# myungsub/meta-interpolation

Measured on AMD Instinct MI355X. Metric: inner-loop steps/sec, higher is better.
Workload: dtype f32 (3x3 convolutions: Winograd F(4x4) / F(2x2) on exact-f32 MFMAs, csrc/winograd4.h + winograd.hip; weight gradients and 5x5 / 7x7 / direct layers on csrc/convk*.hip: bf16x6 split operands, f32 accumulate; 51-tap op on 8-bit frames: exact integer frames x bf16x3 split taps, f32 accumulate); 1 GPU; c2_sepconv_256x448_b4_s5; plugin=sepconv, tasks_per_gpu=4, global_meta_batch=4, inner_steps=5, frame=256x448x3, inner_rule=lslr+SGD, seeded_weights=default, parallelism=task-parallel x1, 1 all-reduce of outer grads

## Files before the change

meta-interpolation_amd/csrc/winograd4.h:

```cpp
#pragma once

namespace w4 {

constexpr int TT = 32;
constexpr int COB = 32;
constexpr int KC = 8;
constexpr int PTS = 36;
constexpr int VBUF = PTS * KC * TT;
constexpr int XBUF = PTS * 16 * TT;
constexpr int LDS_FLOATS = XBUF > 2 * VBUF ? XBUF : 2 * VBUF;
#ifndef SAVFI_W4_MAXC
#define SAVFI_W4_MAXC 512
#endif

__host__ __device__ inline bool use_f4(int K, int I) { return K <= SAVFI_W4_MAXC && I <= SAVFI_W4_MAXC; }
__host__ __device__ inline int kp_of(int K) { return (K + KC - 1) / KC * KC; }
__host__ __device__ inline int ip_of(int I) { return (I + COB - 1) / COB * COB; }

__device__ __forceinline__ void g_rows(const float (&g)[3], float (&t)[6]) {
  const float s = g[0] + g[2];
  const float s4 = fmaf(4.f, g[2], g[0]);
  t[0] = 0.25f * g[0];
  t[1] = (s + g[1]) * (-1.f / 6.f);
  t[2] = (s - g[1]) * (-1.f / 6.f);
  t[3] = fmaf(2.f, g[1], s4) * (1.f / 24.f);
  t[4] = fmaf(-2.f, g[1], s4) * (1.f / 24.f);
  t[5] = g[2];
}

__device__ __forceinline__ void filter_transform_block4(const float* __restrict__ w, float* __restrict__ U, int Co, int Ci, int K, int I,
                                                        int KP, int IP, int mode, int bx, int by) {
  __shared__ __attribute__((aligned(16))) float stage[8 * 18 * 64];
  const int kk = threadIdx.x & 3, ii = threadIdx.x >> 2;
  const int nI = (IP + 63) / 64;
  const int k = 4 * bx + kk, i = 64 * (by % nI) + ii;
  const int task = by / nI;
  w += (size_t)task * Co * Ci * 9;
  U += (size_t)task * PTS * KP * IP;
  float g[3][3];
#pragma unroll
  for (int a = 0; a < 3; ++a)
#pragma unroll
    for (int b = 0; b < 3; ++b) {
      float val = 0.f;
      if (k < K && i < I)
        val = mode == 0 ? w[((size_t)i * Ci + k) * 9 + a * 3 + b] : w[((size_t)k * Ci + i) * 9 + (2 - a) * 3 + (2 - b)];
      g[a][b] = val;
    }
  float t[6][3];
#pragma unroll
  for (int b = 0; b < 3; ++b) {
    const float col[3] = {g[0][b], g[1][b], g[2][b]};
    float o[6];
    g_rows(col, o);
#pragma unroll
    for (int r = 0; r < 6; ++r) t[r][b] = o[r];
  }
  const int cbl = ii >> 5, cb = (ii >> 4) & 1, il = ii & 15;
  const int lane = kk * 16 + il;
#pragma unroll
  for (int r = 0; r < 6; ++r) {
    float o[6];
    g_rows(t[r], o);
#pragma unroll
    for (int c = 0; c < 6; ++c) {
      const int xi = 6 * r + c, wave = xi / 9, v = 2 * (xi % 9) + cb;
      float* blk = stage + (cbl * 4 + wave) * (18 * 64);
      if (v < 16) blk[((v >> 2) * 64 + lane) * 4 + (v & 3)] = o[c];
      else blk[16 * 64 + lane * 2 + (v - 16)] = o[c];
    }
  }
  __syncthreads();
  const int chunk = bx >> 1, s2 = bx & 1, ncob = IP / COB, cob0 = 2 * (by % nI);
  if (4 * bx >= KP) return;
#pragma unroll
  for (int it = 0; it < 8 * 18 * 64 / 4 / 256; ++it) {
    const int e = (it * 256 + threadIdx.x) * 4;
    const int blkid = e / (18 * 64), off = e - blkid * (18 * 64);
    const int cobq = cob0 + (blkid >> 2), wv = blkid & 3;
    if (cobq >= ncob) continue;
    float* dst = U + ((((size_t)chunk * ncob + cobq) * 4 + wv) * 2 + s2) * (18 * 64) + off;
    *reinterpret_cast<f32x4*>(dst) = *reinterpret_cast<const f32x4*>(stage + e);
  }
}

struct W4Args {
  const float* x;
  const float* U;
  const float* bias;
  float* out;
  int K, I, KP, IP, H, W, Ho, Wo, off, tiles_y, tiles_x;
  float slope;
  int tile_shift;
  int T, N;
  const float* mask;
  float mask_slope;
  int out_unit16;
  int nsplit, chunks_per_split;
  float* partial;
  int flat, ty4, tx4, ntb;
  unsigned tx_mul;
  float* pooled;
  int Hp, Wp;
};

__device__ __forceinline__ i32x4 w4_rsrc(const void* base, unsigned bytes) {
  const unsigned long long p = reinterpret_cast<unsigned long long>(base);
  i32x4 r;
  r.x = (int)(unsigned)p;
  r.y = (int)(unsigned)(p >> 32);
  r.z = (int)bytes;
  r.w = 0x00020000;
  return r;
}

__device__ __forceinline__ i32x4 w4_uniform(i32x4 r) {
  r.x = __builtin_amdgcn_readfirstlane(r.x); r.y = __builtin_amdgcn_readfirstlane(r.y);
  r.z = __builtin_amdgcn_readfirstlane(r.z); r.w = __builtin_amdgcn_readfirstlane(r.w);
  return r;
}

__device__ __forceinline__ void bt6(float d0, float d1, float d2, float d3, float d4, float d5, float (&o)[6]) {
  const float a = fmaf(-4.f, d2, d4), b = fmaf(-4.f, d1, d3);
  const float c = d4 - d2, e = d3 - d1;
  o[0] = fmaf(4.f, d0, fmaf(-5.f, d2, d4));
  o[1] = a + b;
  o[2] = a - b;
  o[3] = fmaf(2.f, e, c);
  o[4] = fmaf(-2.f, e, c);
  o[5] = fmaf(4.f, d1, fmaf(-5.f, d3, d5));
}

__device__ __forceinline__ f32x2 w4_fma2(float s, f32x2 x, f32x2 y) { return __builtin_elementwise_fma((f32x2){s, s}, x, y); }
__device__ __forceinline__ void bt6p(f32x2 d0, f32x2 d1, f32x2 d2, f32x2 d3, f32x2 d4, f32x2 d5, f32x2 (&o)[6]) {
  const f32x2 a = w4_fma2(-4.f, d2, d4), b = w4_fma2(-4.f, d1, d3);
  const f32x2 c = d4 - d2, e = d3 - d1;
  o[0] = w4_fma2(4.f, d0, w4_fma2(-5.f, d2, d4));
  o[1] = a + b;
  o[2] = a - b;
  o[3] = w4_fma2(2.f, e, c);
  o[4] = w4_fma2(-2.f, e, c);
  o[5] = w4_fma2(4.f, d1, w4_fma2(-5.f, d3, d5));
}

__device__ __forceinline__ void at6(float m0, float m1, float m2, float m3, float m4, float m5, float (&o)[4]) {
  const float s1 = m1 + m2, d1 = m1 - m2, s2 = m3 + m4, d2 = m3 - m4;
  o[0] = m0 + s1 + s2;
  o[1] = fmaf(2.f, d2, d1);
  o[2] = fmaf(4.f, s2, s1);
  o[3] = fmaf(8.f, d2, d1) + m5;
}

__device__ __forceinline__ void at6p(f32x2 m0, f32x2 m1, f32x2 m2, f32x2 m3, f32x2 m4, f32x2 m5, f32x2 (&o)[4]) {
  const f32x2 s1 = m1 + m2, d1 = m1 - m2, s2 = m3 + m4, d2 = m3 - m4;
  o[0] = m0 + s1 + s2;
  o[1] = w4_fma2(2.f, d2, d1);
  o[2] = w4_fma2(4.f, s2, s1);
  o[3] = w4_fma2(8.f, d2, d1) + m5;
}

template <int VECW, int IN16, bool MASK, bool POOL = false>
__global__ __launch_bounds__(256, 2) void wino4_conv3x3(W4Args a) {
  extern __shared__ __attribute__((aligned(16))) float lds[];
  const int tid = threadIdx.x, lane = tid & 63, w = __builtin_amdgcn_readfirstlane(tid >> 6);
  const int j = lane & 15, kg = lane >> 4;

  const int nblk = a.IP / COB;
  int tb, cob, n, sp;
  {
    const unsigned flat = blockIdx.x, nwg = gridDim.x;
    const unsigned ntb = (unsigned)a.ntb;
    const unsigned xcd = flat & 7u, q8 = nwg >> 3, rem = nwg & 7u;
    unsigned item = xcd * q8 + min(xcd, rem) + (flat >> 3);
    cob = (int)(item % (unsigned)nblk);
    item /= (unsigned)nblk;
    tb = (int)(item % ntb);
    item /= ntb;
    sp = (int)(item % (unsigned)a.nsplit);
    n = (int)(item / (unsigned)a.nsplit);
  }
  const int i0 = cob * COB;
  const int task = a.T > 1 ? n % a.T : 0;
  const size_t cplane = (size_t)a.H * a.W;
  const float* xp = a.x + (size_t)n * a.K * cplane;

  const int tl = lane & 31;
  auto tile_of = [&](int tbq, int& ty, int& tx) {
    if (a.flat) {
      const unsigned t = 32u * (unsigned)tbq + (unsigned)tl, tx4 = (unsigned)a.tx4;
      unsigned q = __umulhi(t, a.tx_mul);
      unsigned r = t - q * tx4;
      if (r >= tx4) { ++q; r -= tx4; }
      ty = (int)q;
      tx = (int)r;
      return t < (unsigned)a.ty4 * tx4;
    }
    const int tsh = a.tile_shift, tbw = 1 << tsh, tbh = TT >> tsh;
    const int tby = tbq / a.tiles_x, tbx = tbq - tby * a.tiles_x;
    ty = tby * tbh + (tl >> tsh);
    tx = tbx * tbw + (tl & (tbw - 1));
    return true;
  };

  const int kc = 2 * w + (lane >> 5);
  int tyi, txi;
  const bool live = tile_of(tb, tyi, txi);
  const int y0 = live ? 4 * tyi - a.off : a.H, x0 = live ? 4 * txi - a.off : 0;
  constexpr int WC = IN16 ? IN16 - 1 : 0;
  unsigned pv[6], pn[IN16 ? 6 : 1], pn2[IN16 == 2 ? 6 : 1];
  unsigned long long shl = 0, colm[6] = {~0ull, ~0ull, ~0ull, ~0ull, ~0ull, ~0ull};
  int partial = 0;
  unsigned chunk_bytes;
  unsigned plane_b;
  if constexpr (IN16) {
    plane_b = 64u;
    chunk_bytes = KC * 64u;
    auto at = [&](bool row, int y, int x) {
      return (row && x >= 0 && x < a.W) ? (unsigned)((y * (a.W >> 4) + (x >> 4)) * a.K) * 64u + (unsigned)(x & 15) * 4u + (unsigned)kc * 64u : 0x80000000u;
    };
#pragma unroll
    for (int r = 0; r < 6; ++r) {
      const int y = y0 + r;
      const bool row = y >= 0 && y < a.H;
      pv[r] = at(row, y, x0 + WC);
      pn[IN16 ? r : 0] = at(row, y, x0);
      if constexpr (IN16 == 2) pn2[r] = at(row, y, x0 + 5);
    }
  } else {
    plane_b = (unsigned)cplane * 4u;
    chunk_bytes = KC * plane_b;
    const int xa = x0 < 0 ? 0 : x0;
#pragma unroll
    for (int r = 0; r < 6; ++r) {
      const int y = y0 + r;
      pv[r] = (y >= 0 && y < a.H) ? (unsigned)(y * a.W + xa) * 4u + (unsigned)kc * plane_b : 0x80000000u;
    }
    shl = __builtin_amdgcn_ballot_w64(x0 < 0);
    const unsigned long long all = __builtin_amdgcn_ballot_w64(true);
#pragma unroll
    for (int c = 0; c < 6; ++c) {
      colm[c] = __builtin_amdgcn_ballot_w64(!live || (x0 + c >= 0 && x0 + c < a.W));
      if (colm[c] != all) partial |= 1 << c;
    }
  }
  const int cbeg = sp * a.chunks_per_split;
  const int nch = min(cbeg + a.chunks_per_split, a.KP / KC) - cbeg;
  const unsigned sample_bytes = (unsigned)a.K * (unsigned)cplane * 4u;
  auto xrs = [&](int c) {
    c = (c < nch - 1 ? c : nch - 1) + cbeg;
    const unsigned first = (unsigned)c * chunk_bytes;
    return w4_rsrc(reinterpret_cast<const char*>(xp) + first, sample_bytes - first);
  };

  float d[6][6];
  auto load_wide = [&](const i32x4& rs) {
#pragma unroll
    for (int r = 0; r < 6; ++r) {
      const f32x4 v = savfi_raw_buffer_load_x4(rs, (int)pv[r], 0, 0);
      d[r][WC] = v.x; d[r][WC + 1] = v.y; d[r][WC + 2] = v.z; d[r][WC + 3] = v.w;
    }
  };
  auto load_narrow = [&](const i32x4& rs) {
#pragma unroll
    for (int r = 0; r < 6; ++r) {
      if constexpr (IN16 == 3) {
        const f32x2 v = savfi_raw_buffer_load_x2(rs, (int)pn[r], 0, 0);
        d[r][0] = v.x; d[r][1] = v.y;
      } else if constexpr (IN16 == 2) {
        d[r][0] = savfi_raw_buffer_load_x1(rs, (int)pn[r], 0, 0);
        d[r][5] = savfi_raw_buffer_load_x1(rs, (int)pn2[r], 0, 0);
      } else {
        const f32x2 v = savfi_raw_buffer_load_x2(rs, (int)pv[r] + 16, 0, 0);
        d[r][4] = v.x; d[r][5] = v.y;
      }
    }
  };
  const bool edge = !IN16 && (shl != 0 || partial != 0);
  auto fix_patch = [&]() {
    if (shl != 0) {
      if (a.off == 1) {
#pragma unroll
        for (int r = 0; r < 6; ++r)
#pragma unroll
          for (int c = 5; c >= 1; --c) asm volatile("v_cndmask_b32 %0, %0, %1, %2" : "+v"(d[r][c]) : "v"(d[r][c - 1]), "s"(shl));
      } else if (a.off == 2) {
#pragma unroll
        for (int r = 0; r < 6; ++r)
#pragma unroll
          for (int c = 5; c >= 2; --c) asm volatile("v_cndmask_b32 %0, %0, %1, %2" : "+v"(d[r][c]) : "v"(d[r][c - 2]), "s"(shl));
      }
    }
#pragma unroll
    for (int c = 0; c < 6; ++c)
      if (partial & (1 << c)) {
#pragma unroll
        for (int r = 0; r < 6; ++r) asm volatile("v_cndmask_b32 %0, 0, %0, %1" : "+v"(d[r][c]) : "s"(colm[c]));
      }
  };
  const int vw = (((kc >> 2) * 4 + (kc & 3)) * 16 + (tl & 15)) * 2 + (tl >> 4);
  f32x2 tp[6][3];
  auto pk_cols = [&](int cp) {
    f32x2 o[6];
    bt6p((f32x2){d[0][2 * cp], d[0][2 * cp + 1]}, (f32x2){d[1][2 * cp], d[1][2 * cp + 1]}, (f32x2){d[2][2 * cp], d[2][2 * cp + 1]},
         (f32x2){d[3][2 * cp], d[3][2 * cp + 1]}, (f32x2){d[4][2 * cp], d[4][2 * cp + 1]}, (f32x2){d[5][2 * cp], d[5][2 * cp + 1]}, o);
#pragma unroll
    for (int r = 0; r < 6; ++r) tp[r][cp] = o[r];
  };
  auto row_out = [&](int rp, float* vdst) {
    float o[6];
    bt6(tp[rp][0].x, tp[rp][0].y, tp[rp][1].x, tp[rp][1].y, tp[rp][2].x, tp[rp][2].y, o);
#pragma unroll
    for (int c = 0; c < 6; ++c) vdst[vw + (6 * rp + c) * 256] = o[c];
  };
  auto load_row = [&](const i32x4& rs, int r) {
    const f32x4 v = savfi_raw_buffer_load_x4(rs, (int)pv[r], 0, 0);
    d[r][WC] = v.x; d[r][WC + 1] = v.y; d[r][WC + 2] = v.z; d[r][WC + 3] = v.w;
    if constexpr (IN16 == 3) {
      const f32x2 u = savfi_raw_buffer_load_x2(rs, (int)pn[r], 0, 0);
      d[r][0] = u.x; d[r][1] = u.y;
    } else if constexpr (IN16 == 2) {
      d[r][0] = savfi_raw_buffer_load_x1(rs, (int)pn[r], 0, 0);
      d[r][5] = savfi_raw_buffer_load_x1(rs, (int)pn2[r], 0, 0);
    } else {
      const f32x2 u = savfi_raw_buffer_load_x2(rs, (int)pv[r] + 16, 0, 0);
      d[r][4] = u.x; d[r][5] = u.y;
    }
  };

  f32x4 acc[9][2][2];
#pragma unroll
  for (int q = 0; q < 9; ++q)
#pragma unroll
    for (int cb = 0; cb < 2; ++cb)
#pragma unroll
      for (int t = 0; t < 2; ++t) acc[q][cb][t] = (f32x4){0.f, 0.f, 0.f, 0.f};
  const unsigned ubytes = (unsigned)PTS * (unsigned)a.KP * (unsigned)a.IP * 4u;
  const i32x4 urs = w4_rsrc(a.U + (size_t)task * PTS * a.KP * a.IP, ubytes);
  const unsigned ulane4 = (unsigned)lane * 16u, ulane2 = 16u * 64u * 4u + (unsigned)lane * 8u;
  auto u_of = [&](int c, int s) {
    c = (c < nch - 1 ? c : nch - 1) + cbeg;
    return ((((unsigned)c * (unsigned)nblk + (unsigned)cob) * 4u + (unsigned)w) * 2u + (unsigned)s) * (18u * 64u * 4u);
  };
  f32x4 a4[4];
  f32x2 a2;
  auto load_a4 = [&](int b, unsigned uo) { a4[b] = savfi_raw_buffer_load_x4(urs, (int)(ulane4 + (unsigned)b * 1024u), (int)uo, 0); };
  auto load_a2 = [&](unsigned uo) { a2 = savfi_raw_buffer_load_x2(urs, (int)ulane2, (int)uo, 0); };
  const int vr = (9 * w * 8 + kg) * 32 + 2 * j;

  {
    const i32x4 rs = xrs(0);
    load_wide(rs);
    load_narrow(rs);
  }
  load_a4(0, u_of(0, 0)); load_a4(1, u_of(0, 0)); load_a4(2, u_of(0, 0)); load_a4(3, u_of(0, 0)); load_a2(u_of(0, 0));
  if (edge) fix_patch();
#pragma unroll
  for (int cp = 0; cp < 3; ++cp) pk_cols(cp);
#pragma unroll
  for (int r = 0; r < 6; ++r) row_out(r, lds);
  {
    const i32x4 rs = xrs(1);
    load_wide(rs);
    load_narrow(rs);
  }
  __builtin_amdgcn_s_waitcnt(0);
  __syncthreads();

  const bool half_last = cbeg + nch == a.KP / KC && a.K - (a.KP - KC) <= 4;
  auto chunk = [&](int ch, const float* vcur, float* vnext, auto last_tag) {
    constexpr bool last = decltype(last_tag)::value;
    f32x2 bq[3];
    bq[0] = *reinterpret_cast<const f32x2*>(vcur + vr);
    bq[1] = *reinterpret_cast<const f32x2*>(vcur + vr + 256);
    const i32x4 rs2 = xrs(ch + 2);
#pragma unroll
    for (int g = 0; g < 18; ++g) {
      const int s = g / 9, q = g % 9;
      if (last && g == 9 && half_last) break;
      if (g + 2 < 18) {
        const int s2 = (g + 2) / 9, q2 = (g + 2) % 9;
        bq[(g + 2) % 3] = *reinterpret_cast<const f32x2*>(vcur + vr + q2 * 256 + s2 * 128);
      }
#pragma unroll
      for (int cb = 0; cb < 2; ++cb) {
        const int v = 2 * q + cb;
        const float av = v < 16 ? a4[v >> 2][v & 3] : a2[v - 16];
#pragma unroll
        for (int t = 0; t < 2; ++t) {
          acc[q][cb][t] = __builtin_amdgcn_mfma_f32_16x16x4f32(av, bq[g % 3][t], acc[q][cb][t], 0, 0, 0);
        }
      }
      const unsigned un = s == 0 ? u_of(ch, 1) : u_of(ch + 1, 0);
      if (q == 1 || q == 3 || q == 5 || q == 7) load_a4(q >> 1, un);
      if (q == 8) load_a2(un);
      if (!last) {
        if (g == 9 && edge) fix_patch();
        if (g >= 9 && g < 12) pk_cols(g - 9);
        if (g >= 12) { row_out(g - 12, vnext); load_row(rs2, g - 12); }
      }
      __builtin_amdgcn_sched_barrier(0);
    }
  };
  for (int ch = 0; ch < nch - 1; ++ch) {
    const int cur = ch & 1;
    chunk(ch, lds + cur * VBUF, lds + (cur ^ 1) * VBUF, std::false_type{});
    __syncthreads();
  }
  chunk(nch - 1, lds + ((nch - 1) & 1) * VBUF, lds, std::true_type{});
  __builtin_amdgcn_s_waitcnt(0);
  __syncthreads();

  const int split = a.nsplit > 1 ? 1 : 0;
  float* const obase = split ? a.partial + (size_t)sp * a.N * a.I * a.Ho * a.Wo : a.out;
  float bvals[2][2];
#pragma unroll
  for (int cb = 0; cb < 2; ++cb)
#pragma unroll
    for (int qq = 0; qq < 2; ++qq) {
      const int i = i0 + 16 * cb + (tid >> 5) + 8 * qq;
      bvals[cb][qq] = (a.bias && split == 0 && i < a.I) ? a.bias[task * a.I + i] : 0.f;
    }

  const int otl = tid & 31, och = tid >> 5;
  int tbo = tb, oty = tyi, otx = txi;
  bool olive = live;
  if constexpr (!MASK) {
    asm volatile("" : "+s"(tbo));
    olive = tile_of(tbo, oty, otx);
  }
  const int oy = olive ? 4 * oty : a.Ho, ox = 4 * otx;
  const unsigned oplane = (unsigned)(a.Ho * a.Wo) * 4u;
  constexpr int NS = 4 / VECW;
  unsigned ooff[4][NS];
#pragma unroll
  for (int r = 0; r < 4; ++r)
#pragma unroll
    for (int e = 0; e < NS; ++e) {
      const int x = ox + e * VECW;
      const bool ok = oy + r < a.Ho && x < a.Wo;
      if (a.out_unit16) ooff[r][e] = ok ? (unsigned)(((oy + r) * (a.Wo >> 4) + (x >> 4)) * a.I) * 64u + (unsigned)(x & 15) * 4u : 0x80000000u;
      else ooff[r][e] = ok ? (unsigned)((oy + r) * a.Wo + x) * 4u + (unsigned)(lane >> 5) * oplane : 0x80000000u;
    }
  auto pair_rsrc = [&](const float* base, int cb, int qq, unsigned plane_bytes = 0) {
    if (plane_bytes == 0) plane_bytes = oplane;
    const int ie = i0 + 16 * cb + 2 * w + 8 * qq;
    const int have = a.I - ie < 0 ? 0 : (a.I - ie > 2 ? 2 : a.I - ie);
    return w4_rsrc(base + ((size_t)n * a.I + (ie < a.I ? ie : 0)) * (plane_bytes >> 2), (unsigned)have * plane_bytes);
  };
  constexpr int PS = VECW == 4 ? 1 : 2;
  const unsigned pplane = POOL ? (unsigned)(a.Hp * a.Wp) * 4u : 0u;
  unsigned poff[POOL ? 2 : 1][POOL ? PS : 1];
  if constexpr (POOL) {
#pragma unroll
    for (int r = 0; r < 2; ++r)
#pragma unroll
      for (int e = 0; e < PS; ++e) {
        const int py = (oy >> 1) + r, px = (ox >> 1) + e;
        poff[r][e] = (py < a.Hp && px < a.Wp) ? (unsigned)(py * a.Wp + px) * 4u + (unsigned)(lane >> 5) * pplane : 0x80000000u;
      }
  }
  float mk[MASK ? 2 : 1][MASK ? 2 : 1][4][4];
  if constexpr (MASK) {
#pragma unroll
    for (int cb = 0; cb < 2; ++cb)
#pragma unroll
      for (int qq = 0; qq < 2; ++qq) {
        const i32x4 mrs = w4_uniform(pair_rsrc(a.mask, cb, qq));
#pragma unroll
        for (int r = 0; r < 4; ++r)
#pragma unroll
          for (int e = 0; e < NS; ++e) {
            if constexpr (VECW == 4) {
              const f32x4 v = savfi_raw_buffer_load_x4(mrs, (int)ooff[r][e], 0, 0);
              mk[cb][qq][r][0] = v.x; mk[cb][qq][r][1] = v.y; mk[cb][qq][r][2] = v.z; mk[cb][qq][r][3] = v.w;
            } else if constexpr (VECW == 2) {
              const f32x2 v = savfi_raw_buffer_load_x2(mrs, (int)ooff[r][e], 0, 0);
              mk[cb][qq][r][2 * e] = v.x; mk[cb][qq][r][2 * e + 1] = v.y;
            } else {
              mk[cb][qq][r][e] = savfi_raw_buffer_load_x1(mrs, (int)ooff[r][e], 0, 0);
            }
          }
      }
  }
  const float slope = a.slope;
#pragma unroll
  for (int cb = 0; cb < 2; ++cb) {
#pragma unroll
    for (int q = 0; q < 9; ++q)
#pragma unroll
      for (int t = 0; t < 2; ++t)
#pragma unroll
        for (int r = 0; r < 4; ++r)
          lds[((9 * w + q) * 16 + 4 * kg + r) * 32 + ((16 * t + j) ^ (16 * (kg & 1)))] = acc[q][cb][t][r];
    __syncthreads();
    auto finish = [&](auto act_tag) {
      constexpr int ACT = decltype(act_tag)::value;
#pragma unroll
      for (int qq = 0; qq < 2; ++qq) {
        const int chl = och + 8 * qq;
        const int col = otl ^ (16 * ((chl >> 2) & 1));
        f32x2 t4p[4][3];
#pragma unroll
        for (int cp = 0; cp < 3; ++cp) {
          f32x2 m[6], o[4];
#pragma unroll
          for (int r = 0; r < 6; ++r)
            m[r] = (f32x2){lds[((6 * r + 2 * cp) * 16 + chl) * 32 + col], lds[((6 * r + 2 * cp + 1) * 16 + chl) * 32 + col]};
          at6p(m[0], m[1], m[2], m[3], m[4], m[5], o);
#pragma unroll
          for (int r = 0; r < 4; ++r) t4p[r][cp] = o[r];
        }
        const float b = bvals[cb][qq];
        const int i = i0 + 16 * cb + chl;
        const i32x4 ors = w4_uniform(a.out_unit16 ? w4_rsrc(obase + (size_t)n * a.I * a.Ho * a.Wo, (unsigned)a.I * oplane) : pair_rsrc(obase, cb, qq));
        const unsigned choff = a.out_unit16 ? (i < a.I ? (unsigned)i * 64u : 0x40000000u) : 0u;
        i32x4 prs = ors;
        if constexpr (POOL) prs = w4_uniform(pair_rsrc(a.pooled, cb, qq, pplane));
        float ye[4];
#pragma unroll
        for (int r = 0; r < 4; ++r) {
          float y[4];
          at6(t4p[r][0].x, t4p[r][0].y, t4p[r][1].x, t4p[r][1].y, t4p[r][2].x, t4p[r][2].y, y);
#pragma unroll
          for (int c = 0; c < 4; ++c) {
            float v = y[c];
            if constexpr (ACT >= 1) v += b;
            if constexpr (ACT == 2) v = fmaxf(v, 0.f);
            if constexpr (ACT == 3) v = fmaxf(v, 0.f) + slope * fminf(v, 0.f);
            if constexpr (MASK) v = mk[MASK ? cb : 0][MASK ? qq : 0][r][c] > 0.f ? v : v * a.mask_slope;
            y[c] = v;
          }
          if constexpr (VECW == 4) {
            savfi_raw_buffer_store_x4((f32x4){y[0], y[1], y[2], y[3]}, ors, (int)(ooff[r][0] + choff), 0, 0);
          } else if constexpr (VECW == 2) {
            savfi_raw_buffer_store_x2((f32x2){y[0], y[1]}, ors, (int)(ooff[r][0] + choff), 0, 0);
            savfi_raw_buffer_store_x2((f32x2){y[2], y[3]}, ors, (int)(ooff[r][1] + choff), 0, 0);
          } else {
#pragma unroll
            for (int c = 0; c < 4; ++c) savfi_raw_buffer_store_x1(y[c], ors, (int)(ooff[r][c] + choff), 0, 0);
          }
          if constexpr (POOL) {
            if (r % 2 == 0) {
#pragma unroll
              for (int c = 0; c < 4; ++c) ye[c] = y[c];
            } else {
              const float p0 = (((ye[0] + ye[1]) + y[0]) + y[1]) / 4.f, p1 = (((ye[2] + ye[3]) + y[2]) + y[3]) / 4.f;
              if constexpr (VECW == 4) {
                savfi_raw_buffer_store_x2((f32x2){p0, p1}, prs, (int)poff[r >> 1][0], 0, 0);
              } else {
                savfi_raw_buffer_store_x1(p0, prs, (int)poff[r >> 1][0], 0, 0);
                savfi_raw_buffer_store_x1(p1, prs, (int)poff[r >> 1][1], 0, 0);
              }
            }
          }
        }
      }
    };
    if (slope == 1.f || split) {
      if (a.bias == nullptr || split) finish(std::integral_constant<int, 0>{});
      else finish(std::integral_constant<int, 1>{});
    } else if (slope == 0.f) {
      finish(std::integral_constant<int, 2>{});
    } else {
      finish(std::integral_constant<int, 3>{});
    }
    __syncthreads();
  }
}

}
```

Measured before the change: 250.0 inner-loop steps/sec.

## Restructure Winograd F(4x4) epilogue to exchange accumulators via wave-partitioned LDS transpose

Result: faster. 252.6 inner-loop steps/sec (median of 6 runs) (+1.0%).

```diff
diff --git a/meta-interpolation_amd/csrc/winograd4.h b/meta-interpolation_amd/csrc/winograd4.h
--- a/meta-interpolation_amd/csrc/winograd4.h
+++ b/meta-interpolation_amd/csrc/winograd4.h
@@ -185,9 +185,9 @@
   const float* xp = a.x + (size_t)n * a.K * cplane;
 
   const int tl = lane & 31;
-  auto tile_of = [&](int tbq, int& ty, int& tx) {
+  auto tile_of = [&](int tbq, int slot, int& ty, int& tx) {
     if (a.flat) {
-      const unsigned t = 32u * (unsigned)tbq + (unsigned)tl, tx4 = (unsigned)a.tx4;
+      const unsigned t = 32u * (unsigned)tbq + (unsigned)slot, tx4 = (unsigned)a.tx4;
       unsigned q = __umulhi(t, a.tx_mul);
       unsigned r = t - q * tx4;
       if (r >= tx4) { ++q; r -= tx4; }
@@ -197,14 +197,14 @@
     }
     const int tsh = a.tile_shift, tbw = 1 << tsh, tbh = TT >> tsh;
     const int tby = tbq / a.tiles_x, tbx = tbq - tby * a.tiles_x;
-    ty = tby * tbh + (tl >> tsh);
-    tx = tbx * tbw + (tl & (tbw - 1));
+    ty = tby * tbh + (slot >> tsh);
+    tx = tbx * tbw + (slot & (tbw - 1));
     return true;
   };
 
   const int kc = 2 * w + (lane >> 5);
   int tyi, txi;
-  const bool live = tile_of(tb, tyi, txi);
+  const bool live = tile_of(tb, tl, tyi, txi);
   const int y0 = live ? 4 * tyi - a.off : a.H, x0 = live ? 4 * txi - a.off : 0;
   constexpr int WC = IN16 ? IN16 - 1 : 0;
   unsigned pv[6], pn[IN16 ? 6 : 1], pn2[IN16 == 2 ? 6 : 1];
@@ -410,124 +410,148 @@
   __builtin_amdgcn_s_waitcnt(0);
   __syncthreads();
 
+  int olane = lane;
+  asm volatile("" : "+v"(olane));
+  const int oj = olane & 15, okg = olane >> 4;
+  const int ot = w >> 1, oh = w & 1;
   const int split = a.nsplit > 1 ? 1 : 0;
   float* const obase = split ? a.partial + (size_t)sp * a.N * a.I * a.Ho * a.Wo : a.out;
   float bvals[2][2];
 #pragma unroll
   for (int cb = 0; cb < 2; ++cb)
 #pragma unroll
-    for (int qq = 0; qq < 2; ++qq) {
-      const int i = i0 + 16 * cb + (tid >> 5) + 8 * qq;
-      bvals[cb][qq] = (a.bias && split == 0 && i < a.I) ? a.bias[task * a.I + i] : 0.f;
-    }
-
-  const int otl = tid & 31, och = tid >> 5;
-  int tbo = tb, oty = tyi, otx = txi;
-  bool olive = live;
-  if constexpr (!MASK) {
-    asm volatile("" : "+s"(tbo));
-    olive = tile_of(tbo, oty, otx);
-  }
-  const int oy = olive ? 4 * oty : a.Ho, ox = 4 * otx;
+    for (int e = 0; e < 2; ++e) {
+      const int i = i0 + 16 * cb + 4 * okg + 2 * oh + e;
+      bvals[cb][e] = (a.bias && split == 0 && i < a.I) ? a.bias[task * a.I + i] : 0.f;
+    }
+
+  int tbo = tb;
+  asm volatile("" : "+s"(tbo));
   const unsigned oplane = (unsigned)(a.Ho * a.Wo) * 4u;
   constexpr int NS = 4 / VECW;
-  unsigned ooff[4][NS];
-#pragma unroll
-  for (int r = 0; r < 4; ++r)
-#pragma unroll
-    for (int e = 0; e < NS; ++e) {
-      const int x = ox + e * VECW;
-      const bool ok = oy + r < a.Ho && x < a.Wo;
-      if (a.out_unit16) ooff[r][e] = ok ? (unsigned)(((oy + r) * (a.Wo >> 4) + (x >> 4)) * a.I) * 64u + (unsigned)(x & 15) * 4u : 0x80000000u;
-      else ooff[r][e] = ok ? (unsigned)((oy + r) * a.Wo + x) * 4u + (unsigned)(lane >> 5) * oplane : 0x80000000u;
-    }
-  auto pair_rsrc = [&](const float* base, int cb, int qq, unsigned plane_bytes = 0) {
-    if (plane_bytes == 0) plane_bytes = oplane;
-    const int ie = i0 + 16 * cb + 2 * w + 8 * qq;
-    const int have = a.I - ie < 0 ? 0 : (a.I - ie > 2 ? 2 : a.I - ie);
-    return w4_rsrc(base + ((size_t)n * a.I + (ie < a.I ? ie : 0)) * (plane_bytes >> 2), (unsigned)have * plane_bytes);
-  };
   constexpr int PS = VECW == 4 ? 1 : 2;
   const unsigned pplane = POOL ? (unsigned)(a.Hp * a.Wp) * 4u : 0u;
+  constexpr int NO = VECW == 1 ? 1 : NS;
+  unsigned ooff[4][NO];
+  int ocols;
+  auto ooff1 = [&](int r, int c) { return c < ocols ? ooff[r][0] + 4u * (unsigned)c : 0x80000000u; };
   unsigned poff[POOL ? 2 : 1][POOL ? PS : 1];
-  if constexpr (POOL) {
-#pragma unroll
-    for (int r = 0; r < 2; ++r)
-#pragma unroll
-      for (int e = 0; e < PS; ++e) {
-        const int py = (oy >> 1) + r, px = (ox >> 1) + e;
-        poff[r][e] = (py < a.Hp && px < a.Wp) ? (unsigned)(py * a.Wp + px) * 4u + (unsigned)(lane >> 5) * pplane : 0x80000000u;
-      }
-  }
-  float mk[MASK ? 2 : 1][MASK ? 2 : 1][4][4];
-  if constexpr (MASK) {
-#pragma unroll
-    for (int cb = 0; cb < 2; ++cb)
-#pragma unroll
-      for (int qq = 0; qq < 2; ++qq) {
-        const i32x4 mrs = w4_uniform(pair_rsrc(a.mask, cb, qq));
+  {
+    int oty, otx;
+    const bool olive = tile_of(tbo, oj + 16 * ot, oty, otx);
+    const int oy = olive ? 4 * oty : a.Ho, ox = 4 * otx;
+    ocols = a.Wo - ox;
+#pragma unroll
+    for (int r = 0; r < 4; ++r)
+#pragma unroll
+      for (int e = 0; e < NO; ++e) {
+        const int x = ox + e * VECW;
+        const bool ok = oy + r < a.Ho && x < a.Wo;
+        if (a.out_unit16) ooff[r][e] = ok ? (unsigned)(((oy + r) * (a.Wo >> 4) + (x >> 4)) * a.I) * 64u + (unsigned)(x & 15) * 4u : 0x80000000u;
+        else ooff[r][e] = ok ? (unsigned)((oy + r) * a.Wo + x) * 4u + (unsigned)(4 * okg) * oplane : 0x80000000u;
+      }
+    if constexpr (POOL) {
+#pragma unroll
+      for (int r = 0; r < 2; ++r)
+#pragma unroll
+        for (int e = 0; e < PS; ++e) {
+          const int py = (oy >> 1) + r, px = (ox >> 1) + e;
+          poff[r][e] = (py < a.Hp && px < a.Wp) ? (unsigned)(py * a.Wp + px) * 4u + (unsigned)(4 * okg) * pplane : 0x80000000u;
+        }
+    }
+  }
+  auto wave_rsrc = [&](const float* base, int cb, int e, unsigned plane_bytes) {
+    const int ie = i0 + 16 * cb + 2 * oh + e;
+    const int have = a.I - ie < 0 ? 0 : (a.I - ie > 13 ? 13 : a.I - ie);
+    return w4_rsrc(base + ((size_t)n * a.I + (ie < a.I ? ie : 0)) * (plane_bytes >> 2), (unsigned)have * plane_bytes);
+  };
+  float mk[MASK ? 2 : 1][4][4];
+  auto fetch_mask = [&](int cb) {
+    if constexpr (MASK) {
+#pragma unroll
+      for (int ch = 0; ch < 2; ++ch) {
+        const i32x4 mrs = w4_uniform(wave_rsrc(a.mask, cb, ch, oplane));
 #pragma unroll
         for (int r = 0; r < 4; ++r)
 #pragma unroll
           for (int e = 0; e < NS; ++e) {
             if constexpr (VECW == 4) {
               const f32x4 v = savfi_raw_buffer_load_x4(mrs, (int)ooff[r][e], 0, 0);
-              mk[cb][qq][r][0] = v.x; mk[cb][qq][r][1] = v.y; mk[cb][qq][r][2] = v.z; mk[cb][qq][r][3] = v.w;
+              mk[MASK ? ch : 0][r][0] = v.x; mk[MASK ? ch : 0][r][1] = v.y; mk[MASK ? ch : 0][r][2] = v.z; mk[MASK ? ch : 0][r][3] = v.w;
             } else if constexpr (VECW == 2) {
               const f32x2 v = savfi_raw_buffer_load_x2(mrs, (int)ooff[r][e], 0, 0);
-              mk[cb][qq][r][2 * e] = v.x; mk[cb][qq][r][2 * e + 1] = v.y;
+              mk[MASK ? ch : 0][r][2 * e] = v.x; mk[MASK ? ch : 0][r][2 * e + 1] = v.y;
             } else {
-              mk[cb][qq][r][e] = savfi_raw_buffer_load_x1(mrs, (int)ooff[r][e], 0, 0);
+              mk[MASK ? ch : 0][r][e] = savfi_raw_buffer_load_x1(mrs, (int)ooff1(r, e), 0, 0);
             }
           }
       }
-  }
+    }
+  };
+  auto by_wave = [&](auto&& f) {
+    switch (w) {
+      case 0: f(std::integral_constant<int, 0>{}); break;
+      case 1: f(std::integral_constant<int, 1>{}); break;
+      case 2: f(std::integral_constant<int, 2>{}); break;
+      default: f(std::integral_constant<int, 3>{}); break;
+    }
+  };
+  f32x2* const xl = reinterpret_cast<f32x2*>(lds) + olane;
   const float slope = a.slope;
-#pragma unroll
-  for (int cb = 0; cb < 2; ++cb) {
-#pragma unroll
-    for (int q = 0; q < 9; ++q)
-#pragma unroll
-      for (int t = 0; t < 2; ++t)
-#pragma unroll
-        for (int r = 0; r < 4; ++r)
-          lds[((9 * w + q) * 16 + 4 * kg + r) * 32 + ((16 * t + j) ^ (16 * (kg & 1)))] = acc[q][cb][t][r];
-    __syncthreads();
+  auto put = [&](auto cb_tag) {
+    constexpr int cb = decltype(cb_tag)::value;
+    by_wave([&](auto wtag) {
+      constexpr int WV = decltype(wtag)::value;
+#pragma unroll
+      for (int q = 0; q < 9; ++q)
+#pragma unroll
+        for (int p = 0; p < 4; ++p)
+          if (p != WV) xl[((9 * WV + q) * 4 + p) * 64] = (f32x2){acc[q][cb][p >> 1][2 * (p & 1)], acc[q][cb][p >> 1][2 * (p & 1) + 1]};
+    });
+  };
+  auto gather = [&](auto cb_tag, f32x2 (&t4)[4][6]) {
+    constexpr int cb = decltype(cb_tag)::value;
+    by_wave([&](auto wtag) {
+      constexpr int WV = decltype(wtag)::value;
+#pragma unroll
+      for (int c = 0; c < 6; ++c) {
+        f32x2 m[6], o[4];
+#pragma unroll
+        for (int r = 0; r < 6; ++r) {
+          const int xi = 6 * r + c, wp = xi / 9, q = xi % 9;
+          if (wp == WV) m[r] = (f32x2){acc[q][cb][WV >> 1][2 * (WV & 1)], acc[q][cb][WV >> 1][2 * (WV & 1) + 1]};
+          else m[r] = xl[((9 * wp + q) * 4 + WV) * 64];
+        }
+        at6p(m[0], m[1], m[2], m[3], m[4], m[5], o);
+#pragma unroll
+        for (int r = 0; r < 4; ++r) t4[r][c] = o[r];
+      }
+    });
+  };
+  auto store = [&](auto cb_tag, const f32x2 (&t4)[4][6]) {
+    constexpr int cb = decltype(cb_tag)::value;
     auto finish = [&](auto act_tag) {
       constexpr int ACT = decltype(act_tag)::value;
 #pragma unroll
-      for (int qq = 0; qq < 2; ++qq) {
-        const int chl = och + 8 * qq;
-        const int col = otl ^ (16 * ((chl >> 2) & 1));
-        f32x2 t4p[4][3];
-#pragma unroll
-        for (int cp = 0; cp < 3; ++cp) {
-          f32x2 m[6], o[4];
-#pragma unroll
-          for (int r = 0; r < 6; ++r)
-            m[r] = (f32x2){lds[((6 * r + 2 * cp) * 16 + chl) * 32 + col], lds[((6 * r + 2 * cp + 1) * 16 + chl) * 32 + col]};
-          at6p(m[0], m[1], m[2], m[3], m[4], m[5], o);
-#pragma unroll
-          for (int r = 0; r < 4; ++r) t4p[r][cp] = o[r];
-        }
-        const float b = bvals[cb][qq];
-        const int i = i0 + 16 * cb + chl;
-        const i32x4 ors = w4_uniform(a.out_unit16 ? w4_rsrc(obase + (size_t)n * a.I * a.Ho * a.Wo, (unsigned)a.I * oplane) : pair_rsrc(obase, cb, qq));
+      for (int ch = 0; ch < 2; ++ch) {
+        const float b = bvals[cb][ch];
+        const int i = i0 + 16 * cb + 4 * okg + 2 * oh + ch;
+        const i32x4 ors = w4_uniform(a.out_unit16 ? w4_rsrc(obase + (size_t)n * a.I * a.Ho * a.Wo, (unsigned)a.I * oplane) : wave_rsrc(obase, cb, ch, oplane));
         const unsigned choff = a.out_unit16 ? (i < a.I ? (unsigned)i * 64u : 0x40000000u) : 0u;
         i32x4 prs = ors;
-        if constexpr (POOL) prs = w4_uniform(pair_rsrc(a.pooled, cb, qq, pplane));
+        if constexpr (POOL) prs = w4_uniform(wave_rsrc(a.pooled, cb, ch, pplane));
         float ye[4];
 #pragma unroll
         for (int r = 0; r < 4; ++r) {
           float y[4];
-          at6(t4p[r][0].x, t4p[r][0].y, t4p[r][1].x, t4p[r][1].y, t4p[r][2].x, t4p[r][2].y, y);
+          at6(t4[r][0][ch], t4[r][1][ch], t4[r][2][ch], t4[r][3][ch], t4[r][4][ch], t4[r][5][ch], y);
 #pragma unroll
           for (int c = 0; c < 4; ++c) {
             float v = y[c];
             if constexpr (ACT >= 1) v += b;
             if constexpr (ACT == 2) v = fmaxf(v, 0.f);
             if constexpr (ACT == 3) v = fmaxf(v, 0.f) + slope * fminf(v, 0.f);
-            if constexpr (MASK) v = mk[MASK ? cb : 0][MASK ? qq : 0][r][c] > 0.f ? v : v * a.mask_slope;
+            if constexpr (MASK) v = mk[MASK ? ch : 0][r][c] > 0.f ? v : v * a.mask_slope;
             y[c] = v;
           }
           if constexpr (VECW == 4) {
@@ -537,7 +561,7 @@
             savfi_raw_buffer_store_x2((f32x2){y[2], y[3]}, ors, (int)(ooff[r][1] + choff), 0, 0);
           } else {
 #pragma unroll
-            for (int c = 0; c < 4; ++c) savfi_raw_buffer_store_x1(y[c], ors, (int)(ooff[r][c] + choff), 0, 0);
+            for (int c = 0; c < 4; ++c) savfi_raw_buffer_store_x1(y[c], ors, (int)(ooff1(r, c) + choff), 0, 0);
           }
           if constexpr (POOL) {
             if (r % 2 == 0) {
@@ -549,7 +573,7 @@
                 savfi_raw_buffer_store_x2((f32x2){p0, p1}, prs, (int)poff[r >> 1][0], 0, 0);
               } else {
                 savfi_raw_buffer_store_x1(p0, prs, (int)poff[r >> 1][0], 0, 0);
-                savfi_raw_buffer_store_x1(p1, prs, (int)poff[r >> 1][1], 0, 0);
+                savfi_raw_buffer_store_x1(p1, prs, (int)poff[r >> 1][PS - 1], 0, 0);
               }
             }
           }
@@ -564,8 +588,21 @@
     } else {
       finish(std::integral_constant<int, 3>{});
     }
-    __syncthreads();
-  }
-}
-
-}
+  };
+  using R0 = std::integral_constant<int, 0>;
+  using R1 = std::integral_constant<int, 1>;
+  f32x2 t4[4][6];
+  fetch_mask(0);
+  put(R0{});
+  __syncthreads();
+  gather(R0{}, t4);
+  store(R0{}, t4);
+  fetch_mask(1);
+  __syncthreads();
+  put(R1{});
+  __syncthreads();
+  gather(R1{}, t4);
+  store(R1{}, t4);
+}
+
+}
```
